# Ryan21wy/HSIMAE

Measured on AMD Instinct MI355X. Metric: HSI patches/sec (9x9x96, mask 75%) pretrain fwd+bwd, higher is better.
Workload: dtype bf16; 1 GPU; HSIMAE-Base pretrain fwd+bwd, 9x9x96 cubes, per-GPU batch 4096, mask 0.75, bf16 MFMA operands / fp32 accumulate + residual; per_gpu_batch=4096, global_batch=4096, parallelism=dp1

## Files before the change

hsimae_amd/csrc/fused_dec.hip:

```cpp
#include "common.h"
#include "kernels.h"
#include <type_traits>
#include <cstdlib>

#ifdef HS_PHASE_TIMING
__device__ unsigned long long hs_phase_cycles[32];
extern "C" __attribute__((visibility("default"))) int hsimae_debug_phases(unsigned long long* out, int reset) {
    int rc = (int)hipMemcpyFromSymbol(out, HIP_SYMBOL(hs_phase_cycles), sizeof(unsigned long long) * 32);
    if (reset) { unsigned long long z[32] = {0}; rc |= (int)hipMemcpyToSymbol(HIP_SYMBOL(hs_phase_cycles), z, sizeof(z)); }
    return rc;
}
#define PH_DECL unsigned long long ph_t0 = __builtin_readcyclecounter(), ph_acc[8] = {0, 0, 0, 0, 0, 0, 0, 0};
#define PH(i) { const unsigned long long ph_t = __builtin_readcyclecounter(); ph_acc[i] += ph_t - ph_t0; ph_t0 = ph_t; }
#define PH_FLUSH(base) if (threadIdx.x == 0) { for (int i = 0; i < 8; ++i) atomicAdd(&hs_phase_cycles[(base) + i], ph_acc[i]); }
#define PH2_DECL unsigned long long ph_t1 = 0, ph_acc2[8] = {0, 0, 0, 0, 0, 0, 0, 0};
#define PH2_START ph_t1 = __builtin_readcyclecounter();
#define PH2(i) { const unsigned long long ph_t = __builtin_readcyclecounter(); ph_acc2[i] += ph_t - ph_t1; ph_t1 = ph_t; }
#define PH2_FLUSH if (threadIdx.x == 0) { for (int i = 0; i < 8; ++i) atomicAdd(&hs_phase_cycles[24 + i], ph_acc2[i]); }
#else
#define PH_DECL
#define PH(i)
#define PH_FLUSH(base)
#define PH2_DECL
#define PH2_START
#define PH2(i)
#define PH2_FLUSH
#endif

#ifndef HS_NT_D
#define HS_NT_D 1
#endif
#ifndef HS_TOUCH_F
#define HS_TOUCH_F 0
#endif
#ifndef HS_TOUCH_M
#define HS_TOUCH_M 0
#endif
#ifndef HS_DEC_STG_N
#define HS_DEC_STG_N 2
#endif
#ifndef HS_DEC_STG_ATTN
#define HS_DEC_STG_ATTN 5
#endif
#ifndef HS_DEC_STG_MLP
#define HS_DEC_STG_MLP 4
#endif
#ifndef HS_DEC_MLP_PREFETCH
#define HS_DEC_MLP_PREFETCH 2
#endif
#ifndef HS_TOUCH_A
#define HS_TOUCH_A 0
#endif
#ifndef HS_DEC_PRIO
#define HS_DEC_PRIO 0
#endif
#ifndef HS_DEC_CORE_NQ
#define HS_DEC_CORE_NQ 2
#endif
#ifndef HS_DEC_REGEO
#define HS_DEC_REGEO 1
#endif
#ifndef HS_DEC_REGEO_MLP
#define HS_DEC_REGEO_MLP 0
#endif
#ifndef HS_DEC_PRELOOP_WAIT
#define HS_DEC_PRELOOP_WAIT 1
#endif
#ifndef HS_DEC_CORE_STG
#define HS_DEC_CORE_STG 0
#endif

namespace {

constexpr int D = 64, HD = 8, HPD = 192;
constexpr int LU = D + 8;
constexpr int LG = HPD + 8;
constexpr int LX = D + 4;
constexpr int WRM = HPD * LU;
constexpr int NT_ = 512;
constexpr int kDwSlotsMlp = 72, kDwSlotsAttn = 32, kDwSlots = kDwSlotsMlp + kDwSlotsAttn;
constexpr int kVN2W = 0, kVN2B = 64, kVW2B = 128, kVW1B = 192, kVW3B = 960, kVN1W = 1728, kVN1B = 1792, kVPB = 1856, kVQB = 1920,
              kVKB = 1984, kVVB = 2048, kVec = 2112;
constexpr size_t kSlabTileFloats = (size_t)256 * kDwSlots * NT_;
static_assert(kDecSlabFloats == 256ll * (kDwSlots * NT_ + kVec), "kernels.h kDecSlabFloats must cover the slab these kernels write");

constexpr int cmax(int a, int b) { return a > b ? a : b; }

template <int MT>
struct DL {
    static constexpr int R = MT * 16;
    static constexpr int MH = (MT + 3) / 4;
    static constexpr int MHF = (MT + 1) / 2;
    static constexpr int VST = R + 8;
    static constexpr int U_BYTES = R * LU * 2;
    static constexpr int QKV_BYTES = 2 * U_BYTES + D * VST * 2;
    static constexpr int REG2 = cmax(cmax(QKV_BYTES, R * LG * 2), R * LX * 4);
    static constexpr int FWD_TOTAL = U_BYTES + REG2;
    static constexpr int IMGB = R * 64 * 2;
    static constexpr int BWD_ATTN_LDS = 6 * IMGB + 2 * 8 * R * 4 + 8 * HS_DEC_CORE_NQ * 2 * 16 * 16 * 2 + 4 * D * (D + 16) * 2 + 5 * D * 4;
    static_assert(2 * IMGB + 8 * R * 4 >= R * LX * 4, "fp32 staging tile must fit over Ob|DXb|lse");
    static_assert(BWD_ATTN_LDS - 6 * IMGB >= 16 * 64 * 2, "image overrun of the unguarded products must stay inside the allocation");
};
constexpr int TTS = 16;
constexpr int TT_PAIR = 2 * 16 * TTS;
constexpr int TT_WAVE = HS_DEC_CORE_NQ * TT_PAIR;

struct Geo4 { int lane, c16, g, wave, wm, wn; };

template <bool SCALAR_WAVE = true>
__device__ __forceinline__ Geo4 geo() {
    Geo4 q;
    q.lane = threadIdx.x & 63; q.c16 = q.lane & 15; q.g = q.lane >> 4;
    q.wave = SCALAR_WAVE ? __builtin_amdgcn_readfirstlane(threadIdx.x >> 6) : (int)(threadIdx.x >> 6);
    q.wm = q.wave >> 1; q.wn = q.wave & 1;
    return q;
}

typedef __attribute__((address_space(3))) const bf16x8* lds_cb128;
typedef __attribute__((address_space(3))) const float* lds_cf32;

template <int MH, int KS, bool WLDS = false>
__device__ __forceinline__ void mm(const bf16_t* A, int lda, int kofs, const bf16_t* W, int KS_total, int nt0,
                                   int ks0, int mt0, int MT, const Geo4& q, f32x4 (&acc)[MH][2]) {
    bf16x8 b[KS][2];
#pragma unroll
    for (int ks = 0; ks < KS; ++ks)
#pragma unroll
        for (int j = 0; j < 2; ++j) {
            if constexpr (WLDS) b[ks][j] = *(lds_cb128)(W + (((nt0 + j) * KS_total + ks0 + ks) * 64 + q.lane) * 8);
            else b[ks][j] = *reinterpret_cast<const bf16x8*>(W + (((size_t)(nt0 + j) * KS_total + ks0 + ks) * 64 + q.lane) * 8);
        }
#pragma unroll
    for (int ks = 0; ks < KS; ++ks)
#pragma unroll
        for (int mi = 0; mi < MH; ++mi) {
            const int mt = mt0 + mi;
            if (mt < MT) {
                const bf16x8 a = *reinterpret_cast<const bf16x8*>(A + (mt * 16 + q.c16) * lda + kofs + ks * 32 + q.g * 8);
#pragma unroll
                for (int j = 0; j < 2; ++j) acc[mi][j] = mfma16(a, b[ks][j], acc[mi][j]);
            }
        }
}

template <int KS>
struct Fr {
    bf16x8 b[KS][2];
    __device__ __forceinline__ void load(const bf16_t* W, int KS_total, int nt0, int ks0, const Geo4& q) {
#pragma unroll
        for (int ks = 0; ks < KS; ++ks)
#pragma unroll
            for (int j = 0; j < 2; ++j)
                b[ks][j] = *reinterpret_cast<const bf16x8*>(W + (((size_t)(nt0 + j) * KS_total + ks0 + ks) * 64 + q.lane) * 8);
    }
};

template <int MH, int KS, bool SW = false>
__device__ __forceinline__ void mm_f(const bf16_t* A, int lda, int kofs, const Fr<KS>& f, int mt0, int MT, const Geo4& q,
                                     f32x4 (&acc)[MH][2]) {
#pragma unroll
    for (int ks = 0; ks < KS; ++ks)
#pragma unroll
        for (int mi = 0; mi < MH; ++mi) {
            const int mt = mt0 + mi;
            if (mt < MT) {
                const bf16x8 a = *reinterpret_cast<const bf16x8*>(A + (mt * 16 + q.c16) * lda + kofs + ks * 32 + q.g * 8);
#pragma unroll
                for (int j = 0; j < 2; ++j) acc[mi][j] = SW ? mfma16(f.b[ks][j], a, acc[mi][j]) : mfma16(a, f.b[ks][j], acc[mi][j]);
            }
        }
}

template <int MT, bool FROM_LDS, int NTHR = NT_>
__device__ __forceinline__ void ln_rows(const float* src, int Ts, const float* gamma, const float* beta, bf16_t* U,
                                        float* XS, float* copy_out) {
    constexpr int R = MT * 16;
    const int c8 = (threadIdx.x & 7) * 8;
    float gm[8], bt[8];
#pragma unroll
    for (int e = 0; e < 8; ++e) { gm[e] = gamma[c8 + e]; bt[e] = beta[c8 + e]; }
    constexpr int NI = (R * 8 + NTHR - 1) / NTHR;
    float4 ga[FROM_LDS ? 1 : NI], gb[FROM_LDS ? 1 : NI];
    if constexpr (!FROM_LDS) {
// ... 319 lines not shown
        }
#pragma unroll
        for (int j = 0; j < 2; ++j) {
            const f32x4 b = *reinterpret_cast<const f32x4*>(w.pb + (q.wn * 2 + j) * 16 + q.g * 4);
#pragma unroll
            for (int mi = 0; mi < L::MHF; ++mi) xr[mi][j] += b;
        }
        mm_f<L::MHF, 2, true>(U, LU, 0, fp, mt0, MT, q, xr);
        Fr<2> f1, f3;
        f1.load(w.w1, 2, q.wn * 2, 0, q);
        f3.load(w.w3, 2, q.wn * 2, 0, q);
        acc_to_xs<L::MHF, true>(XS, mt0, MT, q, xr);
        lds_barrier();
        PH(3)
        ln_rows<MT, true, 256>(nullptr, p.Ts, w.n2w, w.n2b, U, XS, p.x1 + rb * D);
        lds_barrier();
        PH(4)
        Fr<6> f2;
#pragma unroll
        for (int c = 0; c < 3; ++c) {
            f32x4 h1[L::MHF][2], h3[L::MHF][2];
#pragma unroll
            for (int j = 0; j < 2; ++j) {
                const int col = c * 64 + (q.wn * 2 + j) * 16 + q.g * 4;
                f32x4 b1, b3;
#pragma unroll
                for (int r = 0; r < 4; ++r) {
                    b1[r] = col + r < w.h ? w.w1b[col + r] : 0.f;
                    b3[r] = col + r < w.h ? w.w3b[col + r] : 0.f;
                }
#pragma unroll
                for (int mi = 0; mi < L::MHF; ++mi) { h1[mi][j] = b1; h3[mi][j] = b3; }
            }
            mm_f<L::MHF, 2, true>(U, LU, 0, f1, mt0, MT, q, h1);
            mm_f<L::MHF, 2, true>(U, LU, 0, f3, mt0, MT, q, h3);
            if (c < 2) {
                f1.load(w.w1, 2, (c + 1) * 4 + q.wn * 2, 0, q);
                f3.load(w.w3, 2, (c + 1) * 4 + q.wn * 2, 0, q);
            } else {
                f2.load(w.w2, 6, q.wn * 2, 0, q);
            }
#pragma unroll
            for (int mi = 0; mi < L::MHF; ++mi) {
                const int mt = mt0 + mi;
                if (mt >= MT) continue;
#pragma unroll
                for (int j = 0; j < 2; ++j) {
                    const int col = c * 64 + (q.wn * 2 + j) * 16 + q.g * 4;
                    f32x4 gv;
#pragma unroll
                    for (int r = 0; r < 4; ++r) gv[r] = col + r < w.h ? silu_f(h1[mi][j][r]) * h3[mi][j][r] : 0.f;
                    *reinterpret_cast<bf16x4*>(Gb + (mt * 16 + q.c16) * LG + col) = cvt4(gv);
                }
            }
        }
        lds_barrier();
        PH(5)
#pragma unroll
        for (int j = 0; j < 2; ++j) {
            const f32x4 b = *reinterpret_cast<const f32x4*>(w.w2b + (q.wn * 2 + j) * 16 + q.g * 4);
#pragma unroll
            for (int mi = 0; mi < L::MHF; ++mi) xr[mi][j] += b;
        }
        mm_f<L::MHF, 6, true>(Gb, LG, 0, f2, mt0, MT, q, xr);
        lds_barrier();
        PH(6)
        acc_to_xs<L::MHF, true>(XS, mt0, MT, q, xr);
        lds_barrier();
        store_rows<256>(XS, L::R, p.Ts, p.x2 + rb * D);
        lds_barrier();
        PH(7)
    }
    PH_FLUSH(16)
}

typedef __attribute__((ext_vector_type(4))) short s16x4;
__device__ __forceinline__ f32x4 mfma16k16(bf16x4 a, bf16x4 b, f32x4 c) {
    return __builtin_amdgcn_mfma_f32_16x16x16bf16_1k(__builtin_bit_cast(s16x4, a), __builtin_bit_cast(s16x4, b), c, 0, 0, 0);
}
__device__ __forceinline__ bf16x4 zero4() {
    u32x2 z = {0u, 0u};
    return __builtin_bit_cast(bf16x4, z);
}

struct DecAttnFwdArgs { const float* x; float* x1; bf16_t* o; float* lse; int nsamples, Ts; DecW w; };

template <int MT>
__global__ __launch_bounds__(256, 4) void dec_attn_fwd_kernel(DecAttnFwdArgs p) {
    constexpr int R = MT * 16;
    extern __shared__ __attribute__((aligned(16))) char smem[];
    bf16_t* U = reinterpret_cast<bf16_t*>(smem);
    bf16_t* Oi = U + R * LU;
    const Geo4 q = geo();
    const float sc = 0.35355339059327373f * 1.4426950408889634f;
    constexpr int NPAIR = (MT + 1) / 2;

    {
        const int sample = blockIdx.x;
        const size_t rb = (size_t)sample * p.Ts;
        const DecW& w = p.w;
        bf16x8 fw[3][2];
#pragma unroll
        for (int c = 0; c < 3; ++c)
#pragma unroll
            for (int ks = 0; ks < 2; ++ks)
                fw[c][ks] = *reinterpret_cast<const bf16x8*>(w.qkv + (((size_t)(c * 4 + q.wave) * 2 + ks) * 64 + q.lane) * 8);
        const f32x4 bq4 = *reinterpret_cast<const f32x4*>(w.bqkv + q.wave * 16 + q.g * 4);
        const f32x4 bk4 = *reinterpret_cast<const f32x4*>(w.bqkv + D + q.wave * 16 + q.g * 4);
        const float bv1 = w.bqkv[2 * D + q.wave * 16 + q.c16];
        ln_rows<MT, false, 256>(p.x + rb * D, p.Ts, w.n1w, w.n1b, U, nullptr, nullptr);
        lds_barrier();

        bf16x4 kT[MT], vN[MT];
#pragma unroll
        for (int mt = 0; mt < MT; ++mt) {
            const bf16x8 a0 = *reinterpret_cast<const bf16x8*>(U + (mt * 16 + q.c16) * LU + q.g * 8);
            const bf16x8 a1 = *reinterpret_cast<const bf16x8*>(U + (mt * 16 + q.c16) * LU + 32 + q.g * 8);
            f32x4 aq = bq4, ak = bk4, av = f32x4{bv1, bv1, bv1, bv1};
            aq = mfma16(fw[0][0], a0, aq); aq = mfma16(fw[0][1], a1, aq);
            ak = mfma16(fw[1][0], a0, ak); ak = mfma16(fw[1][1], a1, ak);
            av = mfma16(a0, fw[2][0], av); av = mfma16(a1, fw[2][1], av);
            *reinterpret_cast<bf16x4*>(Oi + (mt * 16 + q.c16) * LU + q.wave * 16 + q.g * 4) = cvt4(aq);
            kT[mt] = cvt4(ak); vN[mt] = cvt4(av);
        }

        constexpr int KMIN = (MT > 4) ? 4 : 0;
        f32x4 cinit[MT - KMIN];
#pragma unroll
        for (int kt = KMIN; kt < MT; ++kt)
#pragma unroll
            for (int r = 0; r < 4; ++r) cinit[kt - KMIN][r] = (kt * 16 + q.g * 4 + r >= p.Ts) ? -INFINITY : 0.f;

#pragma unroll 1
        for (int hh = 0; hh < 2; ++hh) {
            const bool mine = (q.g >> 1) == hh;
            const int head = q.wave * 2 + hh;
#pragma unroll
            for (int qt = 0; qt < MT; ++qt) {
                if (qt * 16 >= p.Ts) continue;
                const int query = qt * 16 + q.c16;
                bf16x4 bq = *reinterpret_cast<const bf16x4*>(Oi + query * LU + q.wave * 16 + q.g * 4);
                if (!mine) bq = zero4();
                f32x4 s[MT];
#pragma unroll
                for (int kt = 0; kt < MT; ++kt)
                    s[kt] = mfma16k16(kT[kt], bq, kt < KMIN ? f32x4{0.f, 0.f, 0.f, 0.f} : cinit[kt < KMIN ? 0 : kt - KMIN]);
                float m = -INFINITY;
#pragma unroll
                for (int kt = 0; kt < MT; ++kt)
#pragma unroll
                    for (int r = 0; r < 4; ++r) m = fmaxf(m, s[kt][r]);
                m = rows_max(m);
                const float nm = -m * sc;
                const f32x2 sc2 = {sc, sc}, nm2 = {nm, nm};
                f32x2 ls2 = {0.f, 0.f};
#pragma unroll
                for (int kt = 0; kt < MT; ++kt)
#pragma unroll
                    for (int r = 0; r < 4; r += 2) {
                        const f32x2 t = __builtin_elementwise_fma(f32x2{s[kt][r], s[kt][r + 1]}, sc2, nm2);
                        const f32x2 e = {__builtin_amdgcn_exp2f(t[0]), __builtin_amdgcn_exp2f(t[1])};
                        s[kt][r] = e[0]; s[kt][r + 1] = e[1];
                        ls2 += e;
                    }
                float lsum = ls2[0] + ls2[1];
                lsum = rows_sum(lsum);
// ... 427 lines not shown
                float du[8], t[8], gm[8];
                float (&xh)[8] = xe[i];
                float (&dyv)[8] = dye[i];
                ld8(XS + row * LX + c8, du);
                ld8(n2w + c8, gm);
                const float mean = red8(xh[0] + xh[1] + xh[2] + xh[3] + xh[4] + xh[5] + xh[6] + xh[7]) * (1.f / D);
                float v = 0.f;
#pragma unroll
                for (int e = 0; e < 8; ++e) { xh[e] -= mean; v += xh[e] * xh[e]; }
                const float rstd = rsqrtf(red8(v) * (1.f / D) + 1e-5f);
                float a = 0.f, b = 0.f;
#pragma unroll
                for (int e = 0; e < 8; ++e) { xh[e] *= rstd; t[e] = du[e] * gm[e]; a += t[e]; b += t[e] * xh[e]; }
                a = red8(a) * (1.f / D); b = red8(b) * (1.f / D);
                float o[8];
#pragma unroll
                for (int e = 0; e < 8; ++e) {
                    o[e] = dyv[e] + rstd * (t[e] - a - xh[e] * b);
                    dgam[e] += du[e] * xh[e];
                    dbet[e] += du[e];
                }
                bst8(rows_rsrc(p.dx1 + rb * D, p.Ts * D * 4), (unsigned)(row * D + c8) * 4u, o);
            }
        }
        lds_barrier();
        PH(4)
    }

    PH_FLUSH(8)
    float* red = XS;
    float* vec = p.slab ? p.slab + kSlabTileFloats + (size_t)blockIdx.x * kVec : nullptr;
    flush_wide(red, dgam, p.g_n2w, p.det, vec ? vec + kVN2W : nullptr);
    flush_wide(red, dbet, p.g_n2b, p.det, vec ? vec + kVN2B : nullptr);
    if (bias_wave && (q.c16 >> 2) == 0) {
#pragma unroll
        for (int c = 0; c < 3; ++c)
#pragma unroll
            for (int t = 0; t < 3; ++t) {
                const int nt12 = (q.wave >> 1) * 3 + t, mat = nt12 >> 2, nt = nt12 & 3;
                const int ci = nt * 16 + q.g * 4 + (q.c16 & 3), col = c * 64 + ci;
                if (mat == 0) {
                    if (c == 0) { if (vec) vec[kVW2B + ci] = dbw[c][t]; else hs_gadd(p.det, p.g_w2b + ci, dbw[c][t]); }
                } else if (col < p.w.h) {
                    if (vec) vec[(mat == 1 ? kVW1B : kVW3B) + col] = dbw[c][t];
                    else hs_gadd(p.det, (mat == 1 ? p.g_w1b : p.g_w3b) + col, dbw[c][t]);
                }
            }
    }
    if (p.slab) {
        float* sl = p.slab + (size_t)blockIdx.x * kDwSlots * NT_ + threadIdx.x;
#pragma unroll
        for (int c = 0; c < 3; ++c)
#pragma unroll
            for (int t = 0; t < 3; ++t)
#pragma unroll
                for (int k2 = 0; k2 < 2; ++k2)
#pragma unroll
                    for (int r = 0; r < 4; ++r) sl[(size_t)(((c * 3 + t) * 2 + k2) * 4 + r) * NT_] = accW[c][t][k2][r];
        return;
    }
#pragma unroll
    for (int c = 0; c < 3; ++c)
#pragma unroll
        for (int t = 0; t < 3; ++t) {
            const int nt12 = (q.wave >> 1) * 3 + t, mat = nt12 >> 2, nt = nt12 & 3;
#pragma unroll
            for (int k2 = 0; k2 < 2; ++k2)
#pragma unroll
                for (int r = 0; r < 4; ++r) {
                    const int n = nt * 16 + q.g * 4 + r, k = ((q.wave & 1) * 2 + k2) * 16 + q.c16;
                    const float v = accW[c][t][k2][r];
                    if (mat == 0) {
                        if (c * 64 + k < p.w.h) hs_gadd(p.det, p.g_w2w + (size_t)n * p.w.h + c * 64 + k, v);
                    } else {
                        float* dst = mat == 1 ? p.g_w1w : p.g_w3w;
                        if (c * 64 + n < p.w.h) hs_gadd(p.det, dst + (size_t)(c * 64 + n) * D + k, v);
                    }
                }
        }
}


template <int MT>
__device__ __forceinline__ void attn_head_bwd(bf16_t* Qb, bf16_t* Kb, bf16_t* Vb, const bf16_t* dOb, const float* lse_h,
                                              const float* dlt_h, bf16_t* T, int head, int Ts, const GeoB& q) {
    const float sc = 0.35355339059327373f * 1.4426950408889634f, scale = 0.35355339059327373f;
    const int rcol = q.c16 * IR + ((((head + (q.g >> 1)) & 7) ^ q.fr) << 3) + (q.g & 1) * 4;
    int rcol2 = rcol;
    asm volatile("" : "+v"(rcol2));
    const int troff = (4 * q.g + q.q4) * IR + ((((head + (q.p4 >> 1)) & 7) ^ q.ft) << 3) + (q.p4 & 1) * 4;
    const int wcol = q.c16 * IR + ((head ^ q.fr) << 3) + (q.g & 1) * 4;
    const int tw = q.c16 * TTS + (((q.g + q.q4) & 3) << 2);
    const int trd = (4 * q.g + q.q4) * TTS + (((q.p4 + q.g) & 3) << 2);
    const f32x4 z4 = {0.f, 0.f, 0.f, 0.f};
    constexpr int KCL = MT > 4 ? 4 : 1;
    const int clamp_from = Ts >> 4;
    f32x4 dkT[MT], dvT[MT];
    bf16x4 KT[MT];
#pragma unroll
    for (int kt = 0; kt < MT; ++kt) {
        dkT[kt] = z4; dvT[kt] = z4;
        KT[kt] = tr4(Kb + kt * 16 * IR + troff);
    }
    auto qtiles = [&](auto nq_tag, int qt0) {
        constexpr int NQ = decltype(nq_tag)::value;
        bf16x4 bq[NQ], bdo[NQ], QT[NQ], dOT[NQ], Bp[NQ], Bds[NQ];
        float lqn[NQ], dl[NQ];
        f32x4 dqT[NQ];
#pragma unroll
        for (int n = 0; n < NQ; ++n) {
            const int qt = qt0 + n, query = qt * 16 + q.c16;
            bq[n] = *reinterpret_cast<const bf16x4*>(Qb + qt * 16 * IR + rcol);
            bdo[n] = *reinterpret_cast<const bf16x4*>(dOb + qt * 16 * IR + rcol2);
            if (q.g >= 2) { bq[n] = zero4(); bdo[n] = zero4(); }
            lqn[n] = -lse_h[query]; dl[n] = dlt_h[query];
            QT[n] = tr4(Qb + qt * 16 * IR + troff);
            dOT[n] = tr4(dOb + qt * 16 * IR + troff);
            dqT[n] = z4; Bp[n] = zero4(); Bds[n] = zero4();
        }
        bf16x4 Kn = *reinterpret_cast<const bf16x4*>(Kb + rcol);
        bf16x4 Vn = *reinterpret_cast<const bf16x4*>(Vb + rcol2);
#pragma unroll
        for (int kt = 0; kt < MT; ++kt) {
            const bf16x4 Kf = Kn, Vf = Vn;
            if (kt + 1 < MT) {
                Kn = *reinterpret_cast<const bf16x4*>(Kb + (kt + 1) * 16 * IR + rcol);
                Vn = *reinterpret_cast<const bf16x4*>(Vb + (kt + 1) * 16 * IR + rcol2);
            }
            f32x4 s[NQ], dp[NQ], pv[NQ], ds[NQ];
#pragma unroll
            for (int n = 0; n < NQ; ++n) {
                s[n] = mfma16k16(Kf, bq[n], z4);
                dp[n] = mfma16k16(Vf, bdo[n], z4);
            }
#pragma unroll
            for (int n = 0; n < NQ; ++n) {
#pragma unroll
#ifdef HS_EXPERIMENT_NOEXP
                for (int r = 0; r < 4; ++r) pv[n][r] = fmaf(s[n][r], sc, lqn[n]);
#else
                for (int r = 0; r < 4; ++r) {
                    const float e = fmaf(s[n][r], sc, lqn[n]);
                    pv[n][r] = __builtin_amdgcn_exp2f((kt >= KCL && clamp_from <= kt) ? fminf(e, 0.f) : e);
                }
#endif
#pragma unroll
                for (int r = 0; r < 4; ++r) ds[n][r] = pv[n][r] * (dp[n][r] - dl[n]);
            }
            if (kt > 0) {
#pragma unroll
                for (int n = 0; n < NQ; ++n) {
                    dkT[kt - 1] = mfma16k16(QT[n], Bds[n], dkT[kt - 1]);
                    dvT[kt - 1] = mfma16k16(dOT[n], Bp[n], dvT[kt - 1]);
                }
            }
#pragma unroll
            for (int n = 0; n < NQ; ++n) {
                const bf16x4 pb = cvt4(pv[n]), dsb = cvt4(ds[n]);
                dqT[n] = mfma16k16(KT[kt], dsb, dqT[n]);
                bf16_t* tp = T + n * TT_PAIR;
                bf16_t* td = tp + 16 * TTS;
                st4(tp + tw, pb);
                st4(td + tw, dsb);
            }
            asm volatile("" ::: "memory");
#pragma unroll
            for (int n = 0; n < NQ; ++n) {
                Bp[n] = tr4(T + n * TT_PAIR + trd);
                Bds[n] = tr4(T + n * TT_PAIR + 16 * TTS + trd);
            }
        }
#pragma unroll
        for (int n = 0; n < NQ; ++n) {
            dkT[MT - 1] = mfma16k16(QT[n], Bds[n], dkT[MT - 1]);
            dvT[MT - 1] = mfma16k16(dOT[n], Bp[n], dvT[MT - 1]);
            if (q.g < 2) {
                bf16x4 v;
#pragma unroll
                for (int r = 0; r < 4; ++r) v[r] = (bf16_t)(dqT[n][r] * scale);
                st4(Qb + (qt0 + n) * 16 * IR + wcol, v);
            }
        }
    };
    if constexpr (HS_DEC_CORE_NQ == 2) {
#pragma unroll 1
        for (int qt = 0; qt + 1 < MT; qt += 2) qtiles(std::integral_constant<int, 2>{}, qt);
        if constexpr (MT & 1) qtiles(std::integral_constant<int, 1>{}, MT - 1);
    } else {
#pragma unroll 1
        for (int qt = 0; qt < MT; ++qt) qtiles(std::integral_constant<int, 1>{}, qt);
    }
    if (q.g < 2) {
#pragma unroll
        for (int kt = 0; kt < MT; ++kt) {
            bf16x4 vk, vv;
            const bool live = kt * 16 + q.c16 < Ts;
#pragma unroll
            for (int r = 0; r < 4; ++r) {
                const float xk = live ? dkT[kt][r] * scale : 0.f, xv = live ? dvT[kt][r] : 0.f;
                vk[r] = (bf16_t)xk; vv[r] = (bf16_t)xv;
            }
            st4(Kb + kt * 16 * IR + wcol, vk);
            st4(Vb + kt * 16 * IR + wcol, vv);
        }
    }
}

struct DecBwdAttnArgs {
    const float* x; const float* dx1; float* dx; const bf16_t* o; const float* lse_g; int nsamples, Ts; DecW w; const bf16_t *qkvT, *pT;
    const float *qf, *kf, *vf, *pf;
    float *g_n1w, *g_n1b, *g_qw, *g_qb, *g_kw, *g_kb, *g_vw, *g_vb, *g_pw, *g_pb;
    HsDet det;
    float* slab;
};

template <int MT>
__global__ __launch_bounds__(512, 2) void dec_bwd_attn_kernel(DecBwdAttnArgs p) {
    using L = DL<MT>;
    constexpr int R = L::R, IMG = R * IR, NPW = (R * 8 + NT_ - 1) / NT_;
    extern __shared__ __attribute__((aligned(16))) char smem[];
    bf16_t* U = reinterpret_cast<bf16_t*>(smem);
    bf16_t* Qb = U + IMG;
    bf16_t* Kb = Qb + IMG;
    bf16_t* Vb = Kb + IMG;
    bf16_t* Ob = Vb + IMG;
    bf16_t* DXb = Ob + IMG;
    float* XS = reinterpret_cast<float*>(Ob);
    float* lse = reinterpret_cast<float*>(DXb + IMG);
    float* dlt = lse + 8 * R;
    bf16_t* TT = reinterpret_cast<bf16_t*>(dlt + 8 * R);
    bf16_t* WQ = TT + 8 * TT_WAVE;
    bf16_t* WP = WQ + 3 * D * LW;
    float* CB = reinterpret_cast<float*>(WP + D * LW);
    GeoB q = geob();
    int wide = ((threadIdx.x & 7) ^ swz(threadIdx.x >> 3)) << 3;
    const int mt0 = q.wm * L::MH;
    int c8 = (threadIdx.x & 7) * 8;
    auto regeo = [&]() { if (HS_DEC_REGEO >= 2) q = geob(fresh_tid()); };
    auto regeo_core = [&]() { if (HS_DEC_REGEO >= 1) q = geob(fresh_tid()); };
    auto rewide = [&]() { if (HS_DEC_REGEO >= 2) { const int t = fresh_tid(); wide = ((t & 7) ^ swz(t >> 3)) << 3; c8 = (t & 7) * 8; } };
    for (int i = threadIdx.x; i < 4 * D * 8; i += NT_) {
        const int m = i / (D * 8), row = (i % (D * 8)) >> 3, k8 = (i & 7) * 8;
        float f[8];
        ld8((m == 0 ? p.qf : (m == 1 ? p.kf : (m == 2 ? p.vf : p.pf))) + (size_t)row * D + k8, f);
        *reinterpret_cast<bf16x8*>(WQ + (m * D + wrow(row)) * LW + k8) = cvt8(f);
    }
    for (int i = threadIdx.x; i < 5 * D; i += NT_) CB[i] = i < 3 * D ? p.w.bqkv[i] : (i < 4 * D ? p.w.n1w[i - 3 * D] : p.w.n1b[i - 4 * D]);
    lds_barrier();

    if (HS_DEC_STG_N > 1) {
        const int n = (int)((blockIdx.x >> 3) % (HS_DEC_STG_N > 1 ? HS_DEC_STG_N : 1)) * HS_DEC_STG_ATTN;
        for (int i = 0; i < n; ++i) __builtin_amdgcn_s_sleep(32);
    }
    if (HS_DEC_PRIO > 0 && q.wave >= 4) __builtin_amdgcn_s_setprio(HS_DEC_PRIO);
    f32x4 accP[2], accQ[3][2];
#pragma unroll
    for (int a = 0; a < 2; ++a) accP[a] = f32x4{0.f, 0.f, 0.f, 0.f};
#pragma unroll
    for (int a = 0; a < 3; ++a)
#pragma unroll
        for (int b = 0; b < 2; ++b) accQ[a][b] = f32x4{0.f, 0.f, 0.f, 0.f};
    float dgam[8], dbet[8], dbpw = 0.f, dbqw[3] = {0.f, 0.f, 0.f};
#pragma unroll
    for (int e = 0; e < 8; ++e) { dgam[e] = 0.f; dbet[e] = 0.f; }
    bf16x8 ones;
#pragma unroll
    for (int e = 0; e < 8; ++e) ones[e] = (bf16_t)1.0f;
    const bool bias_wave = (q.wave & 1) == 0;
    const int r4 = q.c16 & 3;

    float fa[NPW][8], d1a[NPW][8];
    f32x4 l4a;
    bf16x8 ova[NPW];
    auto fetch_sample = [&](int smp, int part = -1) {
        const bool valid = smp < p.nsamples;
        const size_t nb = (size_t)smp * p.Ts;
        const int rbytes = valid ? p.Ts * D * 4 : 0;
        const __amdgpu_buffer_rsrc_t xr = rows_rsrc(p.x + nb * D, rbytes), d1r = rows_rsrc(p.dx1 + nb * D, rbytes);
        const __amdgpu_buffer_rsrc_t orr = rows_rsrc(p.o + nb * D, rbytes >> 1);
        const int tid = fresh_tid();
        const unsigned lo = (unsigned)((tid >> 3) * D + (tid & 7) * 8) * 4u;
#pragma unroll
        for (int i = 0; i < NPW; ++i) {
            const unsigned bo = lo + (unsigned)(i * (NT_ / 8) * D * 4);
            if (part < 0 || part == 0) bld8(xr, bo, fa[i]);
            if (part < 0 || part == 1) bld8(d1r, bo, d1a[i]);
            if (part < 0 || part == 2) ova[i] = __builtin_bit_cast(bf16x8, __builtin_amdgcn_raw_buffer_load_b128(orr, (int)(bo >> 1), 0, 0));
        }
        if (part < 0 || part == 2) {
            l4a = __builtin_bit_cast(f32x4, __builtin_amdgcn_raw_buffer_load_b128(rows_rsrc(p.lse_g + nb * 8, valid ? p.Ts * 32 : 0), tid * 16, 0, 0));
        }
    };
    fetch_sample(blockIdx.x);
    if (HS_DEC_PRELOOP_WAIT) __builtin_amdgcn_s_waitcnt(0x0F70);
    PH_DECL
    PH2_DECL
    for (int sample = blockIdx.x; sample < p.nsamples; sample += gridDim.x) {
        const size_t rb = (size_t)sample * p.Ts;
        const int wl = launder_i(0);
        const bf16_t* WQl = WQ + wl;
        const bf16_t* WPl = WP + wl;
        const float* CBl = CB + wl;
        rewide();
#pragma unroll
        for (int i = 0; i < NPW; ++i) {
            const int pc = threadIdx.x + NT_ * i;
            if (pc < R * 8) {
                const int row = pc >> 3;
                float gm[8], bt[8];
                float (&f)[8] = fa[i];
                float (&d1)[8] = d1a[i];
                const bf16x8 ov = ova[i];
                ld8(CBl + 3 * D + c8, gm); ld8(CBl + 4 * D + c8, bt);
                *reinterpret_cast<bf16x8*>(Ob + row * IR + wide) = ov;
                const float mean = red8(f[0] + f[1] + f[2] + f[3] + f[4] + f[5] + f[6] + f[7]) * (1.f / D);
                float v = 0.f;
#pragma unroll
                for (int e = 0; e < 8; ++e) { f[e] -= mean; v += f[e] * f[e]; }
                const float rstd = rsqrtf(red8(v) * (1.f / D) + 1e-5f);
                float u[8];
#pragma unroll
                for (int e = 0; e < 8; ++e) u[e] = f[e] * rstd * gm[e] + bt[e];
                *reinterpret_cast<bf16x8*>(U + row * IR + wide) = cvt8(u);
                *reinterpret_cast<bf16x8*>(DXb + row * IR + wide) = cvt8(d1);
            }
        }
        if (threadIdx.x < 2 * R) {
            const int row = threadIdx.x >> 1, h4 = (threadIdx.x & 1) * 4;
#pragma unroll
            for (int e = 0; e < 4; ++e) lse[(h4 + e) * R + row] = row < p.Ts ? l4a[e] : 1e30f;
        }
        lds_barrier();
        PH(0)
        regeo();
#pragma unroll
        for (int c = 0; c < 3; ++c) {
            f32x4 acc[L::MH][2];
#pragma unroll
            for (int j = 0; j < 2; ++j) {
                const f32x4 b = *reinterpret_cast<const f32x4*>(CBl + c * D + (q.wn * 2 + j) * 16 + q.g * 4);
#pragma unroll
                for (int mi = 0; mi < L::MH; ++mi) acc[mi][j] = b;
            }
            mm_rows<L::MH, 2>(U, WQl, c * 4 + q.wn * 2, mt0, q, acc);
            bf16_t* dst = c == 0 ? Qb : (c == 1 ? Kb : Vb);
#pragma unroll
            for (int mi = 0; mi < L::MH; ++mi) {
                const int mt = mt0 + mi;
                if (mt >= MT) continue;
#pragma unroll
                for (int j = 0; j < 2; ++j)
                    st4(dst + tile_off(mt, q.wn * 2 + j, q), cvt4(acc[mi][j]));
            }
        }
        PH(1)
        regeo();
        f32x4 dO[L::MH][2];
#pragma unroll
        for (int mi = 0; mi < L::MH; ++mi) { dO[mi][0] = f32x4{0.f, 0.f, 0.f, 0.f}; dO[mi][1] = dO[mi][0]; }
        mm_cols<L::MH>(DXb, WPl, mt0, q, dO);
        f32x4 accb = {0.f, 0.f, 0.f, 0.f};
#pragma unroll 1
        for (int kk = 0; kk < R / 32; ++kk) {
            const bf16x8 a = wg_frag<false>(DXb, q.wave >> 1, kk, q);
            if (bias_wave) accb = mfma16(a, ones, accb);
#pragma unroll
            for (int k2 = 0; k2 < 2; ++k2)
                accP[k2] = mfma16(a, wg_frag<false>(Ob, (q.wave & 1) * 2 + k2, kk, q), accP[k2]);
        }
        if constexpr (R % 32 != 0) {
            const bf16x8 a = wg_frag<true>(DXb, q.wave >> 1, R / 32, q);
            if (bias_wave) accb = mfma16(a, ones, accb);
#pragma unroll
            for (int k2 = 0; k2 < 2; ++k2)
                accP[k2] = mfma16(a, wg_frag<true>(Ob, (q.wave & 1) * 2 + k2, R / 32, q), accP[k2]);
        }
        dbpw += r4 == 0 ? accb[0] : (r4 == 1 ? accb[1] : (r4 == 2 ? accb[2] : accb[3]));
        PH(2)
        regeo();
        bf16x4 dOb16[L::MH][2];
#pragma unroll
        for (int mi = 0; mi < L::MH; ++mi) {
            const int mt = mt0 + mi;
            if (mt >= MT) continue;
#pragma unroll
            for (int j = 0; j < 2; ++j) {
                const int row = mt * 16 + q.c16, col = (q.wn * 2 + j) * 16 + q.g * 4;
                dOb16[mi][j] = cvt4(dO[mi][j]);
                const bf16x4 ob = *reinterpret_cast<const bf16x4*>(Ob + tile_off(mt, q.wn * 2 + j, q));
                float v = bf2f(dOb16[mi][j][0]) * bf2f(ob[0]);
#pragma unroll
                for (int r = 1; r < 4; ++r) v = fmaf(bf2f(dOb16[mi][j][r]), bf2f(ob[r]), v);
                float a = v, b = v;
                swap_rows16(a, b);
                if ((q.g & 1) == 0) dlt[(col >> 3) * R + row] = a + b;
            }
        }
        lds_barrier();
        PH(3)
#pragma unroll
        for (int mi = 0; mi < L::MH; ++mi) {
            const int mt = mt0 + mi;
            if (mt >= MT) continue;
#pragma unroll
            for (int j = 0; j < 2; ++j)
                st4(Ob + tile_off(mt, q.wn * 2 + j, q), dOb16[mi][j]);
        }
        for (int i = threadIdx.x; i < (R - p.Ts) * 16; i += NT_) {
            const int row = p.Ts + (i >> 4), k8 = (i & 7) * 8;
            *reinterpret_cast<bf16x8*>(((i & 8) ? Vb : Kb) + row * IR + k8) = zero8();
        }
        lds_barrier();
        PH(4)
        float touch[4] = {0.f, 0.f, 0.f, 0.f};
        {
            const int nxt = sample + gridDim.x;
            const size_t nb = (size_t)nxt * p.Ts;
            const int t16 = threadIdx.x * 16;
            if (HS_TOUCH_A && nxt < p.nsamples) {
                if (t16 < p.Ts * D) { touch[0] = p.x[nb * D + t16]; touch[1] = p.dx1[nb * D + t16]; }
                if (2 * t16 < p.Ts * D) touch[2] = bf2f(p.o[nb * D + 2 * t16]);
                if (t16 < p.Ts * 8) touch[3] = p.lse_g[nb * 8 + t16];
            }
        }
        if (HS_DEC_CORE_STG > 0 && q.wave >= 4) __builtin_amdgcn_s_sleep(HS_DEC_CORE_STG);
        regeo_core();
        attn_head_bwd<MT>(Qb, Kb, Vb, Ob, lse + q.wave * R, dlt + q.wave * R, TT + q.wave * TT_WAVE, q.wave, p.Ts, q);
        lds_barrier();
        PH(5)
        PH2_START
        __builtin_amdgcn_sched_barrier(0);
        fetch_sample(sample + (int)gridDim.x);
        __builtin_amdgcn_sched_barrier(0);
        PH2(0)
        regeo_core();
        f32x4 du[L::MH][2];
#pragma unroll
        for (int mi = 0; mi < L::MH; ++mi) { du[mi][0] = f32x4{0.f, 0.f, 0.f, 0.f}; du[mi][1] = du[mi][0]; }
        asm volatile("" :: "v"(touch[0]), "v"(touch[1]), "v"(touch[2]), "v"(touch[3]));
        mm_cols<L::MH>(Qb, WQl, mt0, q, du);
        mm_cols<L::MH>(Kb, WQl + D * LW, mt0, q, du);
        mm_cols<L::MH>(Vb, WQl + 2 * D * LW, mt0, q, du);
        PH2(1)
        regeo();
        f32x4 accqb[3];
#pragma unroll
        for (int t = 0; t < 3; ++t) accqb[t] = f32x4{0.f, 0.f, 0.f, 0.f};
#pragma unroll 1
        for (int kk = 0; kk < R / 32; ++kk) {
            bf16x8 b[2];
#pragma unroll
            for (int k2 = 0; k2 < 2; ++k2) b[k2] = wg_frag<false>(U, (q.wave & 1) * 2 + k2, kk, q);
#pragma unroll
            for (int t = 0; t < 3; ++t) {
                const int nt12 = (q.wave >> 1) * 3 + t, mat = nt12 >> 2, nt = nt12 & 3;
                const bf16_t* dOi = mat == 0 ? Qb : (mat == 1 ? Kb : Vb);
                const bf16x8 a = wg_frag<false>(dOi, nt, kk, q);
                if (bias_wave) accqb[t] = mfma16(a, ones, accqb[t]);
#pragma unroll
                for (int k2 = 0; k2 < 2; ++k2) accQ[t][k2] = mfma16(a, b[k2], accQ[t][k2]);
            }
        }
        if constexpr (R % 32 != 0) {
            bf16x8 b[2];
#pragma unroll
            for (int k2 = 0; k2 < 2; ++k2) b[k2] = wg_frag<true>(U, (q.wave & 1) * 2 + k2, R / 32, q);
#pragma unroll
            for (int t = 0; t < 3; ++t) {
                const int nt12 = (q.wave >> 1) * 3 + t, mat = nt12 >> 2, nt = nt12 & 3;
                const bf16_t* dOi = mat == 0 ? Qb : (mat == 1 ? Kb : Vb);
                const bf16x8 a = wg_frag<true>(dOi, nt, R / 32, q);
                if (bias_wave) accqb[t] = mfma16(a, ones, accqb[t]);
#pragma unroll
                for (int k2 = 0; k2 < 2; ++k2) accQ[t][k2] = mfma16(a, b[k2], accQ[t][k2]);
            }
        }
#pragma unroll
        for (int t = 0; t < 3; ++t) dbqw[t] += r4 == 0 ? accqb[t][0] : (r4 == 1 ? accqb[t][1] : (r4 == 2 ? accqb[t][2] : accqb[t][3]));
        PH2(2)
        regeo(); rewide();
        acc_to_xs<L::MH, true>(XS, mt0, MT, q, du);
        float xe[NPW][8], d1e[NPW][8];
#pragma unroll
        for (int i = 0; i < NPW; ++i) {
            const int row = (threadIdx.x + NT_ * i) >> 3;
#pragma unroll
            for (int e = 0; e < 8; ++e) { xe[i][e] = 0.f; d1e[i][e] = 0.f; }
#ifndef HS_ABL_DEC_REREAD
            {
                const unsigned bo = (unsigned)(row * D + c8) * 4u;
                bld8(rows_rsrc(p.x + rb * D, p.Ts * D * 4), bo, xe[i]); bld8(rows_rsrc(p.dx1 + rb * D, p.Ts * D * 4), bo, d1e[i]);
            }
#endif
        }
        PH2(3)
        lds_barrier();
        if (HS_DEC_PRELOOP_WAIT) __builtin_amdgcn_s_waitcnt(0x0F70);
        PH2(4)
        PH(6)
#pragma unroll
        for (int i = 0; i < NPW; ++i) {
            const int pc = threadIdx.x + NT_ * i;
            if (pc < R * 8) {
                const int row = pc >> 3;
                float dv[8], t[8], gm[8];
                float (&xh)[8] = xe[i];
                float (&d1)[8] = d1e[i];
                ld8(XS + row * LX + c8, dv);
                ld8(CBl + 3 * D + c8, gm);
                const float mean = red8(xh[0] + xh[1] + xh[2] + xh[3] + xh[4] + xh[5] + xh[6] + xh[7]) * (1.f / D);
// ... 257 lines not shown
```

Before: 264,100 patches/s.

## Fold LSE and delta subtraction into MFMA via bf16 split-constant K-padding

The attention backward kernel now uses the unused half of the 16-wide K dimension (head dim is 8) in the S and dP MFMAs. There it places a 3-term bf16 split of -lse/sc and -delta against constant ones, so each score comes out already shifted and the per-element fmaf with lse and the delta subtraction go away. LSE and delta are kept in a new interleaved LDS table stored as bf16 splits. The clamp is precomputed as a per-tile limit, and packed f32x2 math and converts are used. This adds precision risk from the 3-term split and changes the LDS layout.

New measurement: 264,100 patches/s. Within noise of the previous version (-0.0%).

```diff
diff --git a/hsimae_amd/csrc/fused_dec.hip b/hsimae_amd/csrc/fused_dec.hip
--- a/hsimae_amd/csrc/fused_dec.hip
+++ b/hsimae_amd/csrc/fused_dec.hip
@@ -97,8 +97,14 @@
     static constexpr int REG2 = cmax(cmax(QKV_BYTES, R * LG * 2), R * LX * 4);
     static constexpr int FWD_TOTAL = U_BYTES + REG2;
     static constexpr int IMGB = R * 64 * 2;
-    static constexpr int BWD_ATTN_LDS = 6 * IMGB + 2 * 8 * R * 4 + 8 * HS_DEC_CORE_NQ * 2 * 16 * 16 * 2 + 4 * D * (D + 16) * 2 + 5 * D * 4;
-    static_assert(2 * IMGB + 8 * R * 4 >= R * LX * 4, "fp32 staging tile must fit over Ob|DXb|lse");
+    static constexpr int SPL_CHUNK = 16 * 64;
+    static constexpr int SPL_CONST = SPL_CHUNK - 8;
+    static constexpr int SPL_BYTES = 8 * SPL_CHUNK * 2;
+    static_assert(2 * R * 4 <= SPL_CONST, "two table rows and the constants must fit in one chunk");
+    static constexpr int BWD_ATTN_LDS = 6 * IMGB + SPL_BYTES + 8 * HS_DEC_CORE_NQ * 2 * 16 * 16 * 2 + 4 * D * (D + 16) * 2 + 5 * D * 4;
+    static_assert(BWD_ATTN_LDS <= 160 * 1024, "one workgroup per CU must fit the 160 KB of LDS");
+    static_assert(R * LX * 4 <= 2 * IMGB + SPL_CONST * 2, "fp32 staging tile must fit over Ob|DXb|table rows and spare the constants");
+    __host__ __device__ static constexpr int spl_off(int row16, int query) { return (row16 >> 1) * SPL_CHUNK + (row16 & 1) * R * 4 + query * 4; }
     static_assert(BWD_ATTN_LDS - 6 * IMGB >= 16 * 64 * 2, "image overrun of the unguarded products must stay inside the allocation");
 };
 constexpr int TTS = 16;
@@ -584,6 +590,20 @@
     u32x2 z = {0u, 0u};
     return __builtin_bit_cast(bf16x4, z);
 }
+__device__ __forceinline__ bf16x4 split3(float x) {
+    bf16x4 v = zero4();
+    v[0] = (bf16_t)x;
+    const float r1 = x - bf2f(v[0]);
+    v[1] = (bf16_t)r1;
+    v[2] = (bf16_t)(r1 - bf2f(v[1]));
+    return v;
+}
+typedef __attribute__((ext_vector_type(2))) __bf16 bf16x2;
+__device__ __forceinline__ bf16x4 cvt22(f32x2 a, f32x2 b) {
+    const u32x2 w = {__builtin_bit_cast(unsigned, __builtin_convertvector(a, bf16x2)), __builtin_bit_cast(unsigned, __builtin_convertvector(b, bf16x2))};
+    return __builtin_bit_cast(bf16x4, w);
+}
+constexpr float kDecSc = 0.35355339059327373f * 1.4426950408889634f;
 
 struct DecAttnFwdArgs { const float* x; float* x1; bf16_t* o; float* lse; int nsamples, Ts; DecW w; };
 
@@ -1177,12 +1197,19 @@
 
 
 template <int MT>
-__device__ __forceinline__ void attn_head_bwd(bf16_t* Qb, bf16_t* Kb, bf16_t* Vb, const bf16_t* dOb, const float* lse_h,
-                                              const float* dlt_h, bf16_t* T, int head, int Ts, const GeoB& q) {
-    const float sc = 0.35355339059327373f * 1.4426950408889634f, scale = 0.35355339059327373f;
-    const int rcol = q.c16 * IR + ((((head + (q.g >> 1)) & 7) ^ q.fr) << 3) + (q.g & 1) * 4;
+__device__ __forceinline__ void attn_head_bwd(bf16_t* Qb, bf16_t* Kb, bf16_t* Vb, const bf16_t* dOb, const bf16_t* spl,
+                                              bf16_t* T, int head, int Ts, const GeoB& q) {
+    using L = DL<MT>;
+    const float sc = kDecSc, scale = 0.35355339059327373f;
+    const int rcol = q.c16 * IR + ((head ^ q.fr) << 3) + (q.g & 1) * 4;
     int rcol2 = rcol;
     asm volatile("" : "+v"(rcol2));
+    const bool dims = q.g < 2;
+    const int spl_k = L::SPL_CONST + (q.g & 1) * 4;
+    const int offK = dims ? rcol : (int)(spl - Kb) + spl_k, offV = dims ? rcol2 : (int)(spl - Vb) + spl_k;
+    const int offQ = dims ? rcol : (int)(spl - Qb) + (q.g == 2 ? L::spl_off(head, q.c16) : spl_k);
+    const int offD = dims ? rcol2 : (int)(spl - dOb) + (q.g == 2 ? L::spl_off(8 + head, q.c16) : spl_k);
+    const int qstep = dims ? 16 * IR : (q.g == 2 ? 64 : 0);
     const int troff = (4 * q.g + q.q4) * IR + ((((head + (q.p4 >> 1)) & 7) ^ q.ft) << 3) + (q.p4 & 1) * 4;
     const int wcol = q.c16 * IR + ((head ^ q.fr) << 3) + (q.g & 1) * 4;
     const int tw = q.c16 * TTS + (((q.g + q.q4) & 3) << 2);
@@ -1190,6 +1217,9 @@
     const f32x4 z4 = {0.f, 0.f, 0.f, 0.f};
     constexpr int KCL = MT > 4 ? 4 : 1;
     const int clamp_from = Ts >> 4;
+    float elim[MT - KCL];
+#pragma unroll
+    for (int kt = KCL; kt < MT; ++kt) elim[kt - KCL] = clamp_from <= kt ? 0.f : __builtin_inff();
     f32x4 dkT[MT], dvT[MT];
     bf16x4 KT[MT];
 #pragma unroll
@@ -1200,29 +1230,27 @@
     auto qtiles = [&](auto nq_tag, int qt0) {
         constexpr int NQ = decltype(nq_tag)::value;
         bf16x4 bq[NQ], bdo[NQ], QT[NQ], dOT[NQ], Bp[NQ], Bds[NQ];
-        float lqn[NQ], dl[NQ];
         f32x4 dqT[NQ];
 #pragma unroll
         for (int n = 0; n < NQ; ++n) {
-            const int qt = qt0 + n, query = qt * 16 + q.c16;
-            bq[n] = *reinterpret_cast<const bf16x4*>(Qb + qt * 16 * IR + rcol);
-            bdo[n] = *reinterpret_cast<const bf16x4*>(dOb + qt * 16 * IR + rcol2);
-            if (q.g >= 2) { bq[n] = zero4(); bdo[n] = zero4(); }
-            lqn[n] = -lse_h[query]; dl[n] = dlt_h[query];
+            const int qt = qt0 + n;
+            bq[n] = *reinterpret_cast<const bf16x4*>(Qb + qt * qstep + offQ);
+            bdo[n] = *reinterpret_cast<const bf16x4*>(dOb + qt * qstep + offD);
             QT[n] = tr4(Qb + qt * 16 * IR + troff);
             dOT[n] = tr4(dOb + qt * 16 * IR + troff);
             dqT[n] = z4; Bp[n] = zero4(); Bds[n] = zero4();
         }
-        bf16x4 Kn = *reinterpret_cast<const bf16x4*>(Kb + rcol);
-        bf16x4 Vn = *reinterpret_cast<const bf16x4*>(Vb + rcol2);
+        bf16x4 Kn = *reinterpret_cast<const bf16x4*>(Kb + offK);
+        bf16x4 Vn = *reinterpret_cast<const bf16x4*>(Vb + offV);
 #pragma unroll
         for (int kt = 0; kt < MT; ++kt) {
             const bf16x4 Kf = Kn, Vf = Vn;
             if (kt + 1 < MT) {
-                Kn = *reinterpret_cast<const bf16x4*>(Kb + (kt + 1) * 16 * IR + rcol);
-                Vn = *reinterpret_cast<const bf16x4*>(Vb + (kt + 1) * 16 * IR + rcol2);
-            }
-            f32x4 s[NQ], dp[NQ], pv[NQ], ds[NQ];
+                Kn = *reinterpret_cast<const bf16x4*>(Kb + (kt + 1) * 16 * IR + offK);
+                Vn = *reinterpret_cast<const bf16x4*>(Vb + (kt + 1) * 16 * IR + offV);
+            }
+            f32x4 s[NQ], dp[NQ];
+            f32x2 pv[NQ][2], ds[NQ][2];
 #pragma unroll
             for (int n = 0; n < NQ; ++n) {
                 s[n] = mfma16k16(Kf, bq[n], z4);
@@ -1231,16 +1259,17 @@
 #pragma unroll
             for (int n = 0; n < NQ; ++n) {
 #pragma unroll
+                for (int h = 0; h < 2; ++h) {
+                    const f32x2 e = f32x2{s[n][2 * h], s[n][2 * h + 1]} * sc;
 #ifdef HS_EXPERIMENT_NOEXP
-                for (int r = 0; r < 4; ++r) pv[n][r] = fmaf(s[n][r], sc, lqn[n]);
+                    pv[n][h] = e;
 #else
-                for (int r = 0; r < 4; ++r) {
-                    const float e = fmaf(s[n][r], sc, lqn[n]);
-                    pv[n][r] = __builtin_amdgcn_exp2f((kt >= KCL && clamp_from <= kt) ? fminf(e, 0.f) : e);
-                }
+                    pv[n][h][0] = __builtin_amdgcn_exp2f(kt >= KCL ? fminf(e[0], elim[kt - KCL]) : e[0]);
+                    pv[n][h][1] = __builtin_amdgcn_exp2f(kt >= KCL ? fminf(e[1], elim[kt - KCL]) : e[1]);
 #endif
-#pragma unroll
-                for (int r = 0; r < 4; ++r) ds[n][r] = pv[n][r] * (dp[n][r] - dl[n]);
+                }
+#pragma unroll
+                for (int h = 0; h < 2; ++h) ds[n][h] = pv[n][h] * f32x2{dp[n][2 * h], dp[n][2 * h + 1]};
             }
             if (kt > 0) {
 #pragma unroll
@@ -1251,7 +1280,7 @@
             }
 #pragma unroll
             for (int n = 0; n < NQ; ++n) {
-                const bf16x4 pb = cvt4(pv[n]), dsb = cvt4(ds[n]);
+                const bf16x4 pb = cvt22(pv[n][0], pv[n][1]), dsb = cvt22(ds[n][0], ds[n][1]);
                 dqT[n] = mfma16k16(KT[kt], dsb, dqT[n]);
                 bf16_t* tp = T + n * TT_PAIR;
                 bf16_t* td = tp + 16 * TTS;
@@ -1321,9 +1350,8 @@
     bf16_t* Ob = Vb + IMG;
     bf16_t* DXb = Ob + IMG;
     float* XS = reinterpret_cast<float*>(Ob);
-    float* lse = reinterpret_cast<float*>(DXb + IMG);
-    float* dlt = lse + 8 * R;
-    bf16_t* TT = reinterpret_cast<bf16_t*>(dlt + 8 * R);
+    bf16_t* SPL = DXb + IMG;
+    bf16_t* TT = SPL + 8 * L::SPL_CHUNK;
     bf16_t* WQ = TT + 8 * TT_WAVE;
     bf16_t* WP = WQ + 3 * D * LW;
     float* CB = reinterpret_cast<float*>(WP + D * LW);
@@ -1341,6 +1369,11 @@
         *reinterpret_cast<bf16x8*>(WQ + (m * D + wrow(row)) * LW + k8) = cvt8(f);
     }
     for (int i = threadIdx.x; i < 5 * D; i += NT_) CB[i] = i < 3 * D ? p.w.bqkv[i] : (i < 4 * D ? p.w.n1w[i - 3 * D] : p.w.n1b[i - 4 * D]);
+    if (threadIdx.x < 16) {
+        bf16x4 c = zero4();
+        if ((threadIdx.x & 1) == 0) { c[0] = (bf16_t)1.0f; c[1] = c[0]; c[2] = c[0]; }
+        st4(SPL + (threadIdx.x >> 1) * L::SPL_CHUNK + L::SPL_CONST + (threadIdx.x & 1) * 4, c);
+    }
     lds_barrier();
 
     if (HS_DEC_STG_N > 1) {
@@ -1423,7 +1456,7 @@
         if (threadIdx.x < 2 * R) {
             const int row = threadIdx.x >> 1, h4 = (threadIdx.x & 1) * 4;
 #pragma unroll
-            for (int e = 0; e < 4; ++e) lse[(h4 + e) * R + row] = row < p.Ts ? l4a[e] : 1e30f;
+            for (int e = 0; e < 4; ++e) st4(SPL + L::spl_off(h4 + e, row), split3((row < p.Ts ? l4a[e] : 1e30f) * (-1.f / kDecSc)));
         }
         lds_barrier();
         PH(0)
@@ -1488,7 +1521,7 @@
                 for (int r = 1; r < 4; ++r) v = fmaf(bf2f(dOb16[mi][j][r]), bf2f(ob[r]), v);
                 float a = v, b = v;
                 swap_rows16(a, b);
-                if ((q.g & 1) == 0) dlt[(col >> 3) * R + row] = a + b;
+                if ((q.g & 1) == 0) st4(SPL + L::spl_off(8 + (col >> 3), row), split3(-(a + b)));
             }
         }
         lds_barrier();
@@ -1520,7 +1553,7 @@
         }
         if (HS_DEC_CORE_STG > 0 && q.wave >= 4) __builtin_amdgcn_s_sleep(HS_DEC_CORE_STG);
         regeo_core();
-        attn_head_bwd<MT>(Qb, Kb, Vb, Ob, lse + q.wave * R, dlt + q.wave * R, TT + q.wave * TT_WAVE, q.wave, p.Ts, q);
+        attn_head_bwd<MT>(Qb, Kb, Vb, Ob, SPL, TT + q.wave * TT_WAVE, q.wave, p.Ts, q);
         lds_barrier();
         PH(5)
         PH2_START
```
